# chg60/phamclust

Measured on AMD Instinct MI355X. Metric: genome-pairs/sec, higher is better.
Workload: dtype int32; 1 GPU; synth(5000,5000) -m peq: full N x N distance-matrix fill; `value` = fills with the genomes resident in HBM and the matrix left in HBM (upload and D2H excluded: see value_wall); n_genomes=5000, n_phams=5000, metric_selector=peq, genome_pairs=12497500, n_genes=531832, n_residues=111773410, parallelism=static pair shard over 1 GPU(s)

## Files before the change

### phamclust_amd/csrc/pc_align.hip

```cpp
#include <numeric>

#include "pc_host.h"

static int small_launch_min() {
    static const int v = [] { const char* e = getenv("PC_SMALL_LAUNCH_MIN"); const int x = e ? atoi(e) : 0; return x > 0 ? x : 192; }();
    return v;
}
static int run_align_classes(pc_ctx* c, const PcTask* task_list, const uint32_t* task_begin , const int32_t* cls_max_lb,
                             uint2* res, hipStream_t st, pc_stats* stats, int ppos) {
    const int nbase = c->ncls_all;
    struct Launch { uint32_t begin, end; int base, mode, max_lb; };
    std::vector<Launch> launches;
    for (int b = 0; b < nbase; ++b) {
        const uint32_t* tb = task_begin + (size_t)b * PC_WAVE_MODES;
        if (tb[PC_WAVE_MODES] == tb[0]) continue;
        const uint32_t n0 = tb[1] - tb[0], n1 = tb[2] - tb[1], n2 = tb[3] - tb[2];
        const int bv = pc_class_variant(b);
        const uint32_t least = (bv >= 0 && pc_nw_variant_w(bv) >= 32) ? 1u : (uint32_t)small_launch_min();
        const bool own2 = n2 >= least, own1 = n1 + (own2 ? 0u : n2) >= least;
        uint32_t at = tb[0];
        const int max_lb = cls_max_lb[b * PC_WAVE_MODES];
        auto put = [&](uint32_t n, int mode) { if (n) launches.push_back({at, at + n, b, mode, max_lb}); at += n; };
        if (own1) { put(n0, PC_MODE_CLASS); put(n1 + (own2 ? 0u : n2), n1 ? PC_MODE_TWO_WAVES : PC_MODE_ONE_WAVE); }
        else put(n0 + n1 + (own2 ? 0u : n2), n0 ? PC_MODE_CLASS : n1 ? PC_MODE_TWO_WAVES : PC_MODE_ONE_WAVE);
// ... 146 lines not shown

static int64_t plan_budget_bytes(pc_ctx* c) {
    if (c->plan_budget > 0) return c->plan_budget;
    size_t free_b = 0, total_b = 0;
    if (hipMemGetInfo(&free_b, &total_b) != hipSuccess) { (void)hipGetLastError(); return (int64_t)16 << 30; }
    const size_t held = c->b_key0.cap + c->b_key1.cap + c->b_val0.cap + c->b_val1.cap + c->b_flags.cap + c->b_excl.cap + c->b_alias.cap +
                        c->b_bucket_row.cap + c->b_res.cap + c->b_sort_tmp.cap;
    return (int64_t)((free_b + held) / 2);
}
static void release_plan_buffers(pc_ctx* c) {
    DevBuf* bufs[] = {&c->b_key0, &c->b_key1, &c->b_val0, &c->b_val1, &c->b_flags, &c->b_excl, &c->b_alias, &c->b_bucket_row, &c->b_res, &c->b_sort_tmp,
                      &c->b_tasks, &c->b_tasks_sorted};
    for (DevBuf* b : bufs) b->release();
}

static int stage_count(pc_ctx* c, int condensed, hipStream_t st, uint64_t tot[3]) {
    PcRange range("pc:count");
    int rc = PC_OK;
    const PcDev& d = c->dev;
    const int64_t Lp = c->shard_pairs;
    if (d.G > 0 && c->min_gene_len == 0) {
        pc_set_error("fill: an empty translation cannot be aligned (aai/peq); the reference fails on it too"); return PC_ERR_DATA;
    }
    if ((rc = c->b_na.ensure((Lp + 1) * 4)) || (rc = c->b_off.ensure((Lp + 1) * 4)) || (rc = c->b_totals.ensure(64))) return rc;
    PC_HIP(hipMemsetAsync(c->b_na.p, 0, (Lp + 1) * 4, st));
    PC_HIP(hipMemsetAsync(c->b_totals.p, 0, 64, st));
    PcWalkArgs a; memset(&a, 0, sizeof(a));
    a.na = c->b_na.as<uint32_t>(); a.totals = c->b_totals.as<unsigned long long>();
    a.as_distance = 0; a.condensed = condensed;
    if ((rc = pc_launch_walk(PCW_COUNT, d, c->shard, a, st))) return rc;
    uint64_t* h_tot = (uint64_t*)(c->h_plan.as<uint32_t>() + 1000);
    PC_HIP(hipMemcpyAsync(h_tot, c->b_totals.p, 24, hipMemcpyDeviceToHost, st));
    PC_HIP(hipStreamSynchronize(st));
    tot[0] = h_tot[0]; tot[1] = h_tot[1]; tot[2] = h_tot[2];
    return PC_OK;
}

static int count_per_target(pc_ctx* c, int condensed, hipStream_t st, std::vector<uint64_t>& per_owned) {
    int rc = PC_OK;
    const int N = c->dev.N;
    if ((rc = c->b_aln_t.ensure((size_t)N * 8))) return rc;
    PC_HIP(hipMemsetAsync(c->b_aln_t.p, 0, (size_t)N * 8, st));
    PcWalkArgs a; memset(&a, 0, sizeof(a));
    a.totals = c->b_totals.as<unsigned long long>() + 5;
    a.aln_t = c->b_aln_t.as<unsigned long long>(); a.condensed = condensed;
    if ((rc = pc_launch_walk(PCW_COUNT, c->dev, c->shard, a, st))) return rc;
    std::vector<uint64_t> all(N);
    PC_HIP(hipMemcpyAsync(all.data(), c->b_aln_t.p, (size_t)N * 8, hipMemcpyDeviceToHost, st));
    PC_HIP(hipStreamSynchronize(st));
// ... 26 lines not shown
    memset(&P.st, 0, sizeof(P.st));
    pc_stats& local = P.st;
    const int64_t base = (rows || groups) ? 0 : c->h_lbase[k0];
    const int64_t Lc = rows ? (int64_t)(k1 - k0) * d.N : groups ? groups->block_slot[k1] - groups->block_slot[k0] : c->h_lbase[k1] - base;
    local.n_pairs = Lc;
    local.n_alignments = (int64_t)A;
    if (A > (uint64_t)PC_PLAN_MAX_ALIGNMENTS) {
        pc_set_error("plan: %llu alignments behind ONE target genome exceed the 2^31-2 a plan can index", (unsigned long long)A); return PC_ERR_LIMIT;
    }
    const int U = d.U;
    const int ncls = c->nlc;
    const int64_t tmp_fixed = std::max<int64_t>(Lc + 1, U + 1);
    if ((rc = c->b_start_q.ensure((U + 1) * 4)) || (rc = c->b_end_q.ensure((U + 1) * 4)) || (rc = c->b_ntask_q.ensure((U + 1) * 4)) ||
        (rc = c->b_task_off_q.ensure((U + 1) * 4)) || (rc = c->b_scan_tmp.ensure(pc_scan_tmp_elems(tmp_fixed) * 4)) || (rc = c->b_plan.ensure(4096)))
        return rc;
    if (Lc > 0 && (rc = pc_scan_exclusive_u32(c->b_na.as<uint32_t>() + base, c->b_off.as<uint32_t>() + base, Lc, c->b_scan_tmp.as<uint32_t>(),
                                              (int64_t)(c->b_scan_tmp.cap / 4), st))) return rc;
    PcWalkArgs a; memset(&a, 0, sizeof(a));
    a.as_distance = 0; a.condensed = condensed;
    a.off = c->b_off.as<uint32_t>();
    uint32_t* const h_plan = c->h_plan.as<uint32_t>();
    uint64_t* h_tot = (uint64_t*)(h_plan + 1000);
    if (A > 0) {
        const int64_t An = (int64_t)A;
        const int key_bits = 2 * d.ubits;
        const size_t sort_bytes = pc_sort_temp_bytes(An, key_bits);
        if ((rc = c->b_key0.ensure(A * 8)) || (rc = c->b_key1.ensure(A * 8)) || (rc = c->b_val0.ensure(A * 4)) || (rc = c->b_val1.ensure(A * 4)) ||
            (rc = c->b_sort_tmp.ensure(std::max<size_t>(sort_bytes, 16))) || (rc = c->b_flags.ensure((A + 1) * 4)) || (rc = c->b_excl.ensure((A + 1) * 4)) ||
            (rc = c->b_alias.ensure(A * 4)) || (rc = c->b_bucket_row.ensure(A * 4)) || (rc = c->b_res.ensure(A * 8)) ||
            (rc = c->b_scan_tmp.ensure(pc_scan_tmp_elems(std::max<int64_t>(tmp_fixed, An + 1)) * 4)))
            return rc;
        const int64_t tmp_elems = (int64_t)(c->b_scan_tmp.cap / 4);
        a.key = c->b_key0.as<unsigned long long>(); a.val = c->b_val0.as<uint32_t>();
        if ((rc = walk_domain(c, PCW_ENUM, rows, groups, k0, k1, a, st))) return rc;
        if ((rc = pc_sort_pairs(c->b_sort_tmp.p, c->b_sort_tmp.cap, c->b_key0.as<unsigned long long>(), c->b_key1.as<unsigned long long>(),
                                c->b_val0.as<uint32_t>(), c->b_val1.as<uint32_t>(), An, key_bits, st))) return rc;
        if ((rc = pc_launch_mark_heads(c->b_key1.as<unsigned long long>(), c->b_flags.as<uint32_t>(), An, st))) return rc;
        if ((rc = pc_scan_exclusive_u32(c->b_flags.as<uint32_t>(), c->b_excl.as<uint32_t>(), An + 1, c->b_scan_tmp.as<uint32_t>(), tmp_elems, st))) return rc;
        PC_HIP(hipMemsetAsync(c->b_start_q.p, 0, (U + 1) * 4, st));
        PC_HIP(hipMemsetAsync(c->b_end_q.p, 0, (U + 1) * 4, st));
        PC_HIP(hipMemsetAsync(c->b_totals.as<unsigned long long>() + 3, 0, 16, st));
        if ((rc = pc_launch_unique(d, c->b_key1.as<unsigned long long>(), c->b_val1.as<uint32_t>(), c->b_flags.as<uint32_t>(), c->b_excl.as<uint32_t>(),
                                   c->b_alias.as<uint32_t>(), c->b_bucket_row.as<int32_t>(), c->b_start_q.as<uint32_t>(), c->b_end_q.as<uint32_t>(),
                                   c->b_totals.as<unsigned long long>(), An, st))) return rc;
        if ((rc = pc_launch_task_count(c->b_start_q.as<uint32_t>(), c->b_end_q.as<uint32_t>(), c->task_plan, c->b_ntask_q.as<uint32_t>(), U, st))) return rc;
        if ((rc = pc_scan_exclusive_u32(c->b_ntask_q.as<uint32_t>(), c->b_task_off_q.as<uint32_t>(), U + 1, c->b_scan_tmp.as<uint32_t>(), tmp_elems, st))) return rc;
        PC_HIP(hipMemcpyAsync(h_plan, c->b_task_off_q.as<uint32_t>() + U, 4, hipMemcpyDeviceToHost, st));
        PC_HIP(hipMemcpyAsync(h_tot, c->b_totals.p, 40, hipMemcpyDeviceToHost, st));
        PC_HIP(hipStreamSynchronize(st));
        const uint32_t ntasks = h_plan[0];
        local.n_tasks = ntasks; local.n_distinct_alignments = (int64_t)h_tot[3]; local.n_distinct_cells = (int64_t)h_tot[4];
        P.ntasks = ntasks; P.n_distinct = (int64_t)h_tot[3];
        int cbits = 1; while ((1 << cbits) < ncls) ++cbits;
        const size_t tb_bytes = pc_sort_temp_bytes((int64_t)std::max<uint32_t>(ntasks, 1), 32 + cbits);
        if ((rc = c->b_tasks.ensure(std::max<uint32_t>(ntasks, 1) * sizeof(PcTask))) || (rc = c->b_tasks_sorted.ensure(std::max<uint32_t>(ntasks, 1) * sizeof(PcTask))) ||
            (rc = c->b_key0.ensure((size_t)ntasks * 8)) || (rc = c->b_key1.ensure((size_t)ntasks * 8)) || (rc = c->b_val0.ensure((size_t)ntasks * 4)) ||
            (rc = c->b_val1.ensure((size_t)ntasks * 4)) || (rc = c->b_sort_tmp.ensure(std::max<size_t>(tb_bytes, 16))))
            return rc;
        if ((rc = pc_launch_task_fill(d, c->b_start_q.as<uint32_t>(), c->b_end_q.as<uint32_t>(), c->task_plan,
// ... 34 lines not shown
        PC_HIP(hipMemsetAsync(res, 0, (size_t)std::max<int64_t>(P.n_distinct, 1) * 8, st));
        task_list = c->b_tasks.as<PcTask>(); tb = sb;
    }
    for (int i = 0; i < ncls; ++i) c->aligned_tasks[i] = tb[i + 1] - tb[i];
    return run_align_classes(c, task_list, tb.data(), c->cls_max_lb.data(), res, st, stats, P.ppos);
}

static int stage_reduce(pc_ctx* c, int metric, int as_distance, const uint2* res, double* out, hipStream_t st, const PcRows* rows = nullptr,
                        const PcGroupsHost* groups = nullptr) {
    PcRange range("pc:reduce");
    pc_ctx::PlanState& P = c->plan;
    if (!P.valid) { pc_set_error("reduce: no plan (pc_plan_dev first)"); return PC_ERR_STATE; }
    PcWalkArgs a; memset(&a, 0, sizeof(a));
    a.off = c->b_off.as<uint32_t>(); a.alias = c->b_alias.as<uint32_t>(); a.res = res; a.out = out;
    a.as_distance = as_distance ? 1 : 0; a.condensed = P.condensed;
    return walk_domain(c, metric == PC_AAI ? PCW_AAI : PCW_PEQ, rows, groups, P.k0, P.k1, a, st);
}

static void add_plan_stats(pc_ctx* c, pc_stats& acc) {
    const pc_stats& ps = c->plan.st;
    acc.n_tasks += ps.n_tasks; acc.n_distinct_alignments += ps.n_distinct_alignments; acc.n_distinct_cells += ps.n_distinct_cells;
    for (size_t i = 0; i < c->aligned_tasks.size() && i < c->last_plan_tasks.size(); ++i) c->last_plan_tasks[i] += c->aligned_tasks[i];
}
static void set_last_plan_tasks(pc_ctx* c, const std::vector<uint32_t>& per_class) {
    c->last_plan_tasks.assign(per_class.begin(), per_class.end());
    c->last_plan_tasks.resize(c->nlc, 0);
    c->last_plan_tasks_valid = true;
}

static int chunk_step(pc_ctx* c, int metric, int ppos, int as_distance, int condensed, double* out, hipStream_t st, int k0, int k1, uint64_t A,
// ... 3 lines not shown
    if (rc == PC_OK) { if (events) PC_HIP(hipEventRecord(c->ev[2], st)); rc = stage_reduce(c, metric, as_distance, c->b_res.as<uint2>(), out, st, rows, groups); }
    if (rc != PC_OK) return rc;
    PC_HIP(hipEventRecord(c->ev[3], st));
    add_plan_stats(c, local);
    if (ms) {
        const hipEvent_t at[4] = {from, c->ev[1], c->ev[2], c->ev[3]};
        PC_HIP(hipEventSynchronize(c->ev[3]));
        for (int i = 0; i < 3; ++i) { float x = 0.f; PC_HIP(hipEventElapsedTime(&x, at[i], at[i + 1])); ms[i] += x; }
    }
    return PC_OK;
}
static int release_for_retry(pc_ctx* c, hipStream_t st, bool slots) {
    PC_HIP(hipStreamSynchronize(st));
    release_plan_buffers(c);
    c->b_scratch.release();
    if (slots) { c->b_na.release(); c->b_off.release(); }
    return PC_OK;
}

int fill_aligned(pc_ctx* c, int metric, int ppos, int as_distance, double* out, int condensed, hipStream_t st, pc_stats& local, bool timed) {
    int rc = PC_OK;
    if ((rc = fill_check_residues(c, "fill", metric))) return rc;
    uint64_t tot[3] = {0, 0, 0};
    c->last_plan_tasks_valid = false;
    c->last_plan_tasks.assign(c->nlc, 0);
    if ((rc = stage_count(c, condensed, st, tot))) return rc;
    local.n_alignments = (int64_t)tot[0]; local.n_cells = (int64_t)tot[1]; local.n_residue_bytes = (int64_t)tot[2];
    const int nown = c->shard.nown;
    const uint64_t A = tot[0];
    uint64_t max_aln = (uint64_t)PC_PLAN_MAX_ALIGNMENTS;
    if (c->plan_budget > 0 || A * PC_PLAN_BYTES_PER_ALIGNMENT > ((uint64_t)1 << 30))
// ... 36 lines not shown
}

static int fill_units_aligned(pc_ctx* c, const PcRows* rows, const PcGroupsHost* groups, int metric, int ppos, int as_distance, double* out,
                              hipStream_t st, pc_stats& local, bool timed) {
    int rc = PC_OK;
    const PcDev& d = c->dev;
    const int U = rows ? rows->nrows : groups->nblocks;
    auto slots = [&](int k0, int k1) { return rows ? (int64_t)(k1 - k0) * d.N : groups->block_slot[k1] - groups->block_slot[k0]; };
    if ((rc = fill_check_residues(c, "fill", metric))) return rc;
    if (d.G > 0 && c->min_gene_len == 0) {
        pc_set_error("fill: an empty translation cannot be aligned (aai/peq); the reference fails on it too"); return PC_ERR_DATA;
    }
    c->last_plan_tasks_valid = false;
    c->last_plan_tasks.assign(c->nlc, 0);
    c->plan.valid = false;
    std::vector<uint64_t> own(U);
    {
        PcRange range("pc:count");
        if ((rc = c->b_totals.ensure(64)) || (rc = c->b_aln_t.ensure((size_t)std::max(U, 1) * 8))) return rc;
        PC_HIP(hipMemsetAsync(c->b_totals.p, 0, 64, st));
        PC_HIP(hipMemsetAsync(c->b_aln_t.p, 0, (size_t)U * 8, st));
        PcWalkArgs a; memset(&a, 0, sizeof(a));
        a.totals = c->b_totals.as<unsigned long long>(); a.aln_t = c->b_aln_t.as<unsigned long long>();
        if ((rc = walk_domain(c, PCW_COUNT, rows, groups, 0, U, a, st))) return rc;
        uint64_t* h_tot = (uint64_t*)(c->h_plan.as<uint32_t>() + 1000);
        PC_HIP(hipMemcpyAsync(h_tot, c->b_totals.p, 24, hipMemcpyDeviceToHost, st));
        PC_HIP(hipMemcpyAsync(own.data(), c->b_aln_t.p, (size_t)U * 8, hipMemcpyDeviceToHost, st));
        PC_HIP(hipStreamSynchronize(st));
        local.n_alignments = (int64_t)h_tot[0]; local.n_cells = (int64_t)h_tot[1]; local.n_residue_bytes = (int64_t)h_tot[2];
    }
// ... 237 lines not shown
```

### phamclust_amd/csrc/pc_common.h

```cpp
#pragma once
#include <hip/hip_runtime.h>
#include <stdint.h>

#define PC_OPEN 11
#define PC_EXT 1
#define PC_NEG (-(1 << 29))
#define PC_PADCODE 255
#define PC_TASK_ROWS 208
#define PC_TASK_BUDGET 49152
#define PC_MAX_W 64

struct PcDev {
    int32_t N, Wb, Wstride, G;
    int32_t U, ubits;
    int32_t n_cu, pad_;
    int64_t E;
    const uint64_t* bitmap;
    const uint32_t* rankpre;
    const int32_t* ent_cnt;
    const int32_t* ent_len;
    const uint2* ent_pair_len;
    const uint2* ent_pair_cnt;
    const uint32_t* sp_end;
    const int32_t* sp_pham;
// ... 230 lines not shown
int pc_launch_affinity_rows_slab(const double* vals, int64_t Lp, const PcRowsSlab& dom, int r0, int n_rows, const int32_t* group, int G, void* state,
                                 int want_gain, hipEvent_t between, hipStream_t st);
int pc_launch_affinity_rows_finish(const void* state, const int32_t* rows, const int32_t* group, const int32_t* goff, const int32_t* qcount, int n_rows, int N,
                                   int G, int invert, void* out, int want_table, int want_gain, hipStream_t st);
struct PcLut { uint8_t v[256]; };
int pc_launch_encode(const uint8_t* raw, const int64_t* seq_off, const int64_t* gene_off, const int32_t* gene_len, const PcLut& lut,
                     uint8_t* codes, int G, hipStream_t st);
int pc_launch_task_keys(const PcDev& d, const PcTask* tasks, unsigned long long* key, uint32_t* val, int ntasks, hipStream_t st);
int pc_launch_task_gather(const PcTask* in, const uint32_t* idx, PcTask* out, int ntasks, hipStream_t st);
size_t pc_sort_temp_bytes(int64_t n, int bits);
int pc_sort_pairs(void* temp, size_t temp_bytes, const unsigned long long* key_in, unsigned long long* key_out, const uint32_t* val_in,
                  uint32_t* val_out, int64_t n, int bits, hipStream_t st);
int pc_launch_mark_heads(const unsigned long long* skey, uint32_t* flags, int64_t n, hipStream_t st);
int pc_launch_unique(const PcDev& d, const unsigned long long* skey, const uint32_t* sval, const uint32_t* flags, const uint32_t* excl,
                     uint32_t* alias, int32_t* bucket_row, uint32_t* start_q, uint32_t* end_q, unsigned long long* totals, int64_t n, hipStream_t st);
int pc_launch_task_count(const uint32_t* start_q, const uint32_t* end_q, const PcTaskPlan& tp, uint32_t* ntask_q, int U, hipStream_t st);
int pc_launch_task_fill(const PcDev& d, const uint32_t* start_q, const uint32_t* end_q, const PcTaskPlan& tp, const uint32_t* task_off_q,
                        PcTask* tasks, int U, hipStream_t st);
int pc_launch_class_bounds(const unsigned long long* sorted_key, int ntasks, int ncls, uint32_t* cls_begin , hipStream_t st);
int pc_launch_task_slice(const PcTask* sorted, int ntasks, const uint32_t* cls_begin, const uint32_t* slice_begin , int rank, int world,
                         PcTask* out, hipStream_t st);
int pc_launch_gather_u32(const uint32_t* src, const int32_t* idx, uint32_t* dst, int n, hipStream_t st);
int pc_launch_assemble(const double* gathered, int world, int64_t stride, int N, double* out, hipStream_t st);
int pc_launch_assemble_table(const double* gathered, int64_t stride, int N, const int32_t* t_rank, const int64_t* t_lbase, double* out, hipStream_t st);
int pc_launch_round6_probe(const double* in, double* out, int64_t n, hipStream_t st);
int pc_launch_unpack_res(const uint2* res, const int32_t* la_plus_lb, int32_t* n_ident, int32_t* n_diag, int64_t n, hipStream_t st);

int pc_nw_num_variants();
int pc_nw_variant_w(int v);
int pc_nw_choose_variant(int lb);
// ... 35 lines not shown
```

### phamclust_amd/csrc/pc_fill_slabs.hip

```cpp
#include <chrono>
#include <climits>

#include "pc_host.h"

#define PC_EDGE_MAX_PAIRS 0x7fffffffLL

namespace {
struct SlabShardScope {
    pc_ctx* c; PcShard shard; int64_t pairs; std::vector<int32_t> owned; std::vector<int64_t> lbase;
    explicit SlabShardScope(pc_ctx* ctx) : c(ctx), shard(ctx->shard), pairs(ctx->shard_pairs), owned(ctx->h_owned), lbase(ctx->h_lbase) {}
    ~SlabShardScope() { c->shard = shard; c->shard_pairs = pairs; c->h_owned.swap(owned); c->h_lbase.swap(lbase); c->plan.valid = false; }
    SlabShardScope(const SlabShardScope&) = delete; SlabShardScope& operator=(const SlabShardScope&) = delete;
};
}

static int64_t pairs_below(int64_t t) { return t * (t - 1) / 2; }

int pc_slab_check(const pc_ctx* c, PcSlabRun& run, const char* what) {
    int rc = PC_OK;
    const char* who = run.who;
    if ((rc = fill_check(c, who, what, &run.metric, nullptr))) return rc;
    if (run.kind == PC_SLAB_NEAREST) {
        if (run.k < 1) { pc_set_error("%s: k %d", who, run.k); return PC_ERR_ARG; }
        if (run.k > PC_NEAREST_MAX_K) { pc_set_error("%s: k %d is above PC_NEAREST_MAX_K = %d", who, run.k, PC_NEAREST_MAX_K); return PC_ERR_LIMIT; }
        run.kk = std::max(std::min(run.k, c->dev.N - 1), 0);
    }
// ... 62 lines not shown
template <class Hook> static int slab_walk(pc_ctx* c, const std::vector<int32_t>& cut, int metric, int as_distance, pc_stats* sum, Hook hook) {
    int rc = PC_OK;
    hipStream_t st = c->stream;
    double* const slab = c->b_edge_slab.as<double>();
    SlabShardScope restore(c);
    std::vector<int32_t> owned; std::vector<int64_t> lbase;
    for (size_t i = 0; i + 1 < cut.size(); ++i) {
        const int t0 = cut[i], t1 = cut[i + 1];
        const int64_t Lp = pairs_below(t1) - pairs_below(t0);
        if (Lp == 0) continue;
        owned.resize((size_t)(t1 - t0)); lbase.resize((size_t)(t1 - t0) + 1);
        for (int t = t0; t < t1; ++t) { owned[t - t0] = t; lbase[t - t0] = pairs_below(t) - pairs_below(t0); }
        lbase[t1 - t0] = Lp;
        if ((rc = wait_last_work(c, st, false))) return rc;
        if ((rc = upload_vec(c->b_edge_owned, owned)) || (rc = upload_vec(c->b_edge_lbase, lbase))) return rc;
        c->plan.valid = false;
        c->shard.nown = t1 - t0; c->shard.ident = 0;
        c->shard.owned = c->b_edge_owned.as<int32_t>(); c->shard.lbase = c->b_edge_lbase.as<int64_t>();
        c->h_owned = owned; c->h_lbase = lbase; c->shard_pairs = Lp;
        pc_stats one; memset(&one, 0, sizeof(one));
        if ((rc = fill_impl(c, metric, as_distance, slab, 0, st, sum ? &one : nullptr))) return rc;
        if (sum) pc_stats_add(*sum, one);
        int64_t hooked_pairs = 0;
        if (const double* const hooked = pc_hooked_slab_values(&hooked_pairs)) {
            if (hooked_pairs != pairs_below(c->dev.N)) {
                pc_set_error("slab walk: pc_hook_slab_values holds %lld values, the triangle of %d genomes has %lld", (long long)hooked_pairs, c->dev.N,
                             (long long)pairs_below(c->dev.N));
                return PC_ERR_ARG;
            }
            PC_HIP(hipMemcpyAsync(slab, hooked + pairs_below(t0), (size_t)Lp * 8, hipMemcpyHostToDevice, st));
        }
// ... 1098 lines not shown
```

### phamclust_amd/csrc/pc_host.h

```cpp
#pragma once
#include <algorithm>
#include <cstdint>
#include <cstdlib>
#include <cstring>
#include <thread>
#include <vector>

#include "pc_common.h"
#include "pc_nw_geometry.h"
#include "../../include/phamclust_hip.h"

struct PcRange {
    bool on;
    explicit PcRange(const char* name);
    ~PcRange();
    PcRange(const PcRange&) = delete; PcRange& operator=(const PcRange&) = delete;
};

constexpr int PC_ERR_NOMEM_INTERNAL = -100;
struct PlanningScope { PlanningScope(); ~PlanningScope(); };
__attribute__((visibility("hidden"))) const double* pc_hooked_slab_values(int64_t* n_pairs);
__attribute__((visibility("hidden"))) const double* pc_hooked_rows_values(int32_t* n_rows, int32_t* n);
struct DevBuf {
    void* p = nullptr; size_t cap = 0;
// ... 100 lines not shown
    DevBuf b_af_group, b_af_member, b_af_goff, b_af_range, b_af_tab, b_af_out, b_af_qcount;
    PinnedBuf h_af;
    int af_ranges = 0;
    float last_af_ms[3] = {0.f, 0.f, 0.f};
    DevBuf b_hist_group, b_hist_state, b_hist_out;
    PinnedBuf h_hist;
    float last_hist_ms[2] = {0.f, 0.f};
    PinnedBuf h_plan;
    struct PlanState {
        bool valid = false; int ppos = 0; int condensed = 1; int64_t A = 0, n_distinct = 0; uint32_t ntasks = 0;
        int k0 = 0, k1 = 0;
        bool whole = false;
        std::vector<uint32_t> tb;
        pc_stats st;
    } plan;
    std::vector<uint32_t> aligned_tasks;
    std::vector<int64_t> last_plan_tasks;
    bool last_plan_tasks_valid = false;
    PinnedBuf h_out;
    float last_align_ms = 0.f;
    hipEvent_t ev[5] = {nullptr, nullptr, nullptr, nullptr, nullptr};
    static constexpr int kAux = 15;
    hipStream_t aux[kAux] = {};
    hipEvent_t aux_ev[kAux + 1] = {};
    int n_streams = 8;
    static constexpr int kLong = 4;
    hipStream_t lng[kLong] = {};
    hipEvent_t lng_ev[kLong] = {};
    int tie_rule = 0;
    int64_t lut_key = -1; const double* lut_ptr = nullptr;
    hipEvent_t ev_last = nullptr;
    bool busy = false;
    hipStream_t last_stream = nullptr;
    int last_set_kernel = -1;
    pc_set_inputs last_set_inputs{};
    pc_set_shape last_set_shape{};
    int64_t plan_budget = 0;
};

struct PcDeviceGuard {
    int prev = -1, dev = -1; bool ok = true;
    explicit PcDeviceGuard(int device) : dev(device) {
        if (hipGetDevice(&prev) != hipSuccess) prev = -1;
        if (prev != dev) {
            hipError_t e = hipSetDevice(dev);
            if (e != hipSuccess) { pc_set_error("hipSetDevice(%d): %s", dev, hipGetErrorString(e)); ok = false; }
        }
    }
    ~PcDeviceGuard() { if (prev >= 0 && prev != dev) (void)hipSetDevice(prev); }
    PcDeviceGuard(const PcDeviceGuard&) = delete;
    PcDeviceGuard& operator=(const PcDeviceGuard&) = delete;
};
#define PC_ON_DEVICE(c) PcDeviceGuard pc_guard_((c)->device); if (!pc_guard_.ok) return PC_ERR_HIP
// ... 209 lines not shown
```

### phamclust_amd/csrc/pc_plan.hip

```cpp
#include <cstring>

#include <rocprim/device/device_radix_sort.hpp>

#include "../../include/phamclust_hip.h"
#include "pc_common.h"
#include "pc_nw_geometry.h"

size_t pc_sort_temp_bytes(int64_t n, int bits) {
    size_t bytes = 0;
    if (n <= 0) return 0;
    hipError_t e = rocprim::radix_sort_pairs(nullptr, bytes, (const unsigned long long*)nullptr, (unsigned long long*)nullptr,
                                             (const uint32_t*)nullptr, (uint32_t*)nullptr, (size_t)n, 0u, (unsigned)bits, (hipStream_t)0);
    return e == hipSuccess ? bytes : 0;
}

int pc_sort_pairs(void* temp, size_t temp_bytes, const unsigned long long* key_in, unsigned long long* key_out, const uint32_t* val_in,
                  uint32_t* val_out, int64_t n, int bits, hipStream_t st) {
    if (n <= 0) return PC_OK;
    hipError_t e = rocprim::radix_sort_pairs(temp, temp_bytes, key_in, key_out, val_in, val_out, (size_t)n, 0u, (unsigned)bits, st);
    if (e != hipSuccess) { pc_set_error("radix_sort_pairs: %s", hipGetErrorString(e)); return PC_ERR_HIP; }
    return PC_OK;
}

__global__ __launch_bounds__(256) void k_mark_heads(const unsigned long long* __restrict__ skey, uint32_t* __restrict__ flags, int64_t n) {
// ... 36 lines not shown
    }
    for (int o = 32; o > 0; o >>= 1) { cells += __shfl_down(cells, o); heads += __shfl_down(heads, o); }
    if ((threadIdx.x & 63) == 0 && heads) { atomicAdd(&red[0], heads); atomicAdd(&red[1], cells); }
    __syncthreads();
    if (threadIdx.x < 2 && red[threadIdx.x]) atomicAdd(&totals[3 + threadIdx.x], red[threadIdx.x]);
}
int pc_launch_unique(const PcDev& d, const unsigned long long* skey, const uint32_t* sval, const uint32_t* flags, const uint32_t* excl,
                     uint32_t* alias, int32_t* bucket_row, uint32_t* start_q, uint32_t* end_q, unsigned long long* totals, int64_t n, hipStream_t st) {
    if (n <= 0) return PC_OK;
    hipLaunchKernelGGL(k_unique, dim3((unsigned)((n + 255) / 256)), dim3(256), 0, st, d, skey, sval, flags, excl, alias, bucket_row, start_q, end_q, totals, n);
    hipError_t e = hipGetLastError();
    if (e != hipSuccess) { pc_set_error("k_unique launch: %s", hipGetErrorString(e)); return PC_ERR_HIP; }
    return PC_OK;
}

__device__ __forceinline__ uint32_t pc_split(const PcTaskPlan& tp, int q, uint32_t n, uint32_t& rem_class) {
    const uint32_t nseg = tp.q_nseg[q], r = nseg > 1 ? n % nseg : 0u;
    rem_class = r ? tp.rem_class[(size_t)q * 16 + r] : 255u;
    return rem_class != 255u ? n - r : n;
}
__global__ void k_task_count(const uint32_t* __restrict__ start_q, const uint32_t* __restrict__ end_q, PcTaskPlan tp,
                             uint32_t* __restrict__ ntask_q, int U) {
    const int q = blockIdx.x * blockDim.x + threadIdx.x;
    if (q > U) return;
    uint32_t nt = 0;
    if (q < U) {
        const uint32_t n = end_q[q] - start_q[q], per = (uint32_t)tp.task_rows[q];
        uint32_t rc; const uint32_t nmain = pc_split(tp, q, n, rc);
        nt = (nmain + per - 1) / per + (rc != 255u ? 1u : 0u);
    }
// ... 112 lines not shown
```

### phamclust_amd/csrc/pc_upload.hip

```cpp
#include <atomic>
#include <chrono>
#include <cstdio>
#include <mutex>
#include <numeric>

#include "pc_host.h"

static void build_code_lut(uint8_t lut[256]) {
    static const char alpha[] = "ARNDCQEGHILKMFPSTWYVBZX*";
    int assigned[256];
    for (int i = 0; i < 256; ++i) assigned[i] = -1;
    for (int k = 0; k < 24; ++k) assigned[(unsigned char)alpha[k]] = k;
    int next = 24;
    for (int v = 0; v < 256; ++v) {
        if (v >= 'a' && v <= 'z') continue;
        if (assigned[v] < 0) assigned[v] = next++;
    }
    for (int v = 'a'; v <= 'z'; ++v) assigned[v] = assigned[v - 32];
    for (int i = 0; i < 256; ++i) lut[i] = (uint8_t)assigned[i];
}

static int apply_shard(pc_ctx* c, int rank, int world) {
    c->plan.valid = false;
    const int N = c->dev.N;
    std::vector<int32_t> owned; std::vector<int64_t> lbase;
    c->h_t_rank.assign(std::max(N, 1), 0); c->h_t_lbase.assign(std::max(N, 1), 0);
    int64_t best = 0;
    for (int r = 0; r < world; ++r) {
        int64_t tot = 0;
        for (int j = 0;; ++j) {
            const int pos = (j & 1) ? world - 1 - r : r;
            const int64_t t = (int64_t)j * world + pos;
            if (t >= N) { if ((int64_t)j * world >= N) break; else continue; }
            if (r == rank) { owned.push_back((int32_t)t); lbase.push_back(tot); }
            c->h_t_rank[t] = r; c->h_t_lbase[t] = tot;
            tot += t;
        }
        if (r == rank) { lbase.push_back(tot); c->shard_pairs = tot; }
// ... 21 lines not shown
    }
    const int64_t G64 = g->gene_off[N];
    if (G64 < 0 || G64 > 0x7fffffffLL || g->gene_off[0] != 0 || (G64 > 0 && (!g->gene_pham || !g->residues))) {
        pc_set_error("pc_upload: bad gene table"); return PC_ERR_ARG;
    }
    const int G = (int)G64;
    static const bool timing = getenv("PC_UPLOAD_TIMING") != nullptr;
    auto tick = std::chrono::steady_clock::now();
    auto lap = [&](const char* what) {
        if (!timing) return;
        auto now = std::chrono::steady_clock::now();
        fprintf(stderr, "pc_upload %-22s %7.1f ms\n", what, std::chrono::duration<double, std::milli>(now - tick).count());
        tick = now;
    };
    if ((rc = wait_last_work(c, nullptr, false))) return rc;
    c->uploaded = false; c->residues_ready = false; c->target_cost.clear(); c->plan.valid = false;
    PC_HIP(hipStreamSynchronize(c->stream));
    if (c->b_scratch.cap > ((size_t)512 << 20)) c->b_scratch.release();

    const int Wstride = W | 1;
    size_t off = 0;
    auto place = [&](size_t bytes) { const size_t at = off; off = (off + bytes + 255) & ~(size_t)255; return at; };
    const size_t o_bitmap = place((size_t)N * Wstride * 8), o_rankpre = place((size_t)N * W * 4), o_gene_len = place((size_t)std::max(G, 1) * 4),
                 o_ent_off = place(((size_t)N + 1) * 4), o_nph = place((size_t)N * 4), o_ngen = place((size_t)N * 4), o_tlen = place((size_t)N * 8);
    const size_t o_ent = off;
    const size_t cap_bytes = o_ent + 6 * (((size_t)std::max(G, 1) * 4 + 255) & ~(size_t)255) + (((size_t)N + 1) * 4 + 255) + (size_t)std::max(P, 1) * 4 + 1024;
    if ((rc = c->h_stage.ensure(cap_bytes))) return rc;
    uint8_t* hs = c->h_stage.as<uint8_t>();
    uint64_t* bitmap = (uint64_t*)(hs + o_bitmap); uint32_t* rankpre = (uint32_t*)(hs + o_rankpre); int32_t* gene_len_h = (int32_t*)(hs + o_gene_len);
    uint32_t* ent_off = (uint32_t*)(hs + o_ent_off); int32_t* nph_h = (int32_t*)(hs + o_nph); int32_t* ngen_h = (int32_t*)(hs + o_ngen);
    int64_t* tlen_h = (int64_t*)(hs + o_tlen);
// ... 165 lines not shown
    const int N = g->n_genomes;
    const int G = c->dev.G;
    if (N != c->dev.N || g->gene_off[N] != (int64_t)G || g->seq_off[G] - g->seq_off[0] != c->n_residue_bytes_in) {
        pc_set_error("pc_upload_residues: not the genomes pc_upload_sets was given (N %d/%d, genes %lld/%d)", N, c->dev.N, (long long)g->gene_off[N], G);
        return PC_ERR_ARG;
    }
    static const bool timing = getenv("PC_UPLOAD_TIMING") != nullptr;
    auto tick = std::chrono::steady_clock::now();
    auto lap = [&](const char* what) {
        if (!timing) return;
        auto now = std::chrono::steady_clock::now();
        fprintf(stderr, "pc_upload %-22s %7.1f ms\n", what, std::chrono::duration<double, std::milli>(now - tick).count());
        tick = now;
    };
    if ((rc = wait_last_work(c, nullptr, false))) return rc;
    c->residues_ready = false; c->plan.valid = false;
    PC_HIP(hipStreamSynchronize(c->stream));
    const std::vector<int32_t>& gene_len = c->h_gene_len;
    const int maxlen = c->max_gene_len;
    std::vector<int64_t> gene_off(G);
    int64_t code_bytes = 0;
    for (int k = 0; k < G; ++k) { gene_off[k] = code_bytes; code_bytes += ((int64_t)gene_len[k] + 15) & ~15LL; }
    std::vector<uint64_t> ghash(std::max(G, 1));
    std::vector<uint8_t> godd(std::max(G, 1), 0);
    uint8_t lut[256]; build_code_lut(lut);
    uint8_t is_odd[256];
    for (int v = 0; v < 256; ++v) is_odd[v] = (uint8_t)(lut[v] >= 24);
    const uint8_t* raw = g->residues;
    const int64_t raw_bytes = g->seq_off[G] - g->seq_off[0];
    static const int64_t stage_max = getenv("PC_RAW_STAGE_MAX") ? atoll(getenv("PC_RAW_STAGE_MAX")) : ((int64_t)512 << 20);
    const bool staged = raw_bytes > 0 && raw_bytes <= stage_max;
// ... 284 lines not shown
    std::vector<int64_t> t_lbase(std::max(N, 1), 0), fill(world, 0);
    std::vector<int32_t> owned; std::vector<int64_t> lbase;
    for (int t = 0; t < N; ++t) {
        const int r = t_rank[t];
        t_lbase[t] = fill[r];
        if (r == rank) { owned.push_back(t); lbase.push_back(fill[r]); }
        fill[r] += t;
    }
    lbase.push_back(fill[rank]);
    c->shard_pairs = fill[rank];
    c->shard_stride = *std::max_element(fill.begin(), fill.end());
    c->rank = rank; c->world = world; c->balanced = true;
    if ((rc = upload_vec(c->b_owned, owned)) || (rc = upload_vec(c->b_lbase, lbase)) || (rc = upload_vec(c->b_t_rank, t_rank)) ||
        (rc = upload_vec(c->b_t_lbase, t_lbase))) return rc;
    c->h_t_rank = t_rank; c->h_t_lbase = t_lbase;
    c->h_owned = owned; c->h_lbase = lbase; c->plan.valid = false;
    c->shard.nown = (int32_t)owned.size();
    c->shard.ident = world == 1 ? 1 : 0;
    c->shard.owned = c->b_owned.as<int32_t>();
    c->shard.lbase = c->b_lbase.as<int64_t>();
    return PC_OK;
}
extern "C" int pc_shard_table(const pc_ctx* c, int32_t* t_rank, int64_t* t_lbase) {
    if (!c || !c->uploaded) { pc_set_error("pc_shard_table: upload first"); return PC_ERR_STATE; }
    if (!t_rank || !t_lbase) { pc_set_error("pc_shard_table: NULL argument"); return PC_ERR_ARG; }
    memcpy(t_rank, c->h_t_rank.data(), sizeof(int32_t) * (size_t)c->dev.N);
    memcpy(t_lbase, c->h_t_lbase.data(), sizeof(int64_t) * (size_t)c->dev.N);
    return PC_OK;
}
extern "C" int pc_target_costs(const pc_ctx* c, uint64_t* cost) {
    if (!c || !c->uploaded) { pc_set_error("pc_target_costs: upload first"); return PC_ERR_STATE; }
// ... 8 lines not shown
```

### phamclust_amd/csrc/pc_walk.hip

```cpp
#include "pc_pairs.h"

#define WCH 32

struct PcPairAcc {
    uint32_t k;
    int64_t cons;
    double num;
    int64_t den;
    int any;
    __device__ __forceinline__ void reset() { k = 0; cons = 0; num = 0.0; den = 0; any = 0; }
};

template <int MODE>
__device__ __forceinline__ void pc_visit(const PcDev& d, const PcWalkArgs& a, PcPairAcc& p, uint32_t es, uint32_t et,
                                         unsigned long long& cells, unsigned long long& rbytes) {
    p.any = 1;
    if (MODE == PCW_POCP) { p.cons += d.ent_cnt[es] + d.ent_cnt[et]; return; }
    if (MODE == PCW_AF) { p.cons += d.ent_len[es] + d.ent_len[et]; return; }
    const int cs = d.ent_cnt[es], ct = d.ent_cnt[et];
    const bool swap = cs > ct;
    const uint32_t ea = swap ? et : es, eb = swap ? es : et;
    const int ca = swap ? ct : cs, cb = swap ? cs : ct;
    const int a0 = d.ent_gene[ea], b0 = d.ent_gene[eb];
    if (MODE == PCW_COUNT) {
// ... 4 lines not shown
        rbytes += la * cb + lb * ca;
    } else if (MODE == PCW_ENUM) {
        for (int ia = 0; ia < ca; ++ia) {
            const unsigned long long qa = d.gene_q[a0 + ia];
            for (int ib = 0; ib < cb; ++ib) {
                const uint32_t k = p.k++;
                a.key[k] = ((unsigned long long)d.gene_q[b0 + ib] << d.ubits) | qa;
                a.val[k] = k;
            }
        }
    } else {
        if (MODE == PCW_PEQ) p.cons += d.ent_len[es] + d.ent_len[et];
        for (int ia = 0; ia < ca; ++ia) {
            double best = -1.0; uint32_t best_len = 0;
            for (int ib = 0; ib < cb; ++ib) {
                const uint2 r = a.res[a.alias[p.k++]];
                const double x = (double)r.x / (double)r.y;
                if (x >= best) { best = x; best_len = r.y; }
            }
            p.num = p.num + best * (double)best_len;
            p.den += best_len;
        }
    }
}

template <int MODE>
__device__ __forceinline__ void pc_walk_word(const PcDev& d, const PcWalkArgs& a, PcPairAcc& acc, uint64_t sw, uint64_t tw, uint32_t bs, uint32_t bt,
                                             unsigned long long& cells, unsigned long long& rbytes) {
    uint64_t x = sw & tw;
    while (x) {
        const int b = __ffsll((long long)x) - 1;
// ... 355 lines not shown
```

Baseline: 25.21 million genome-pairs/s.

## Cache pair counts across fills, fuse unique pass, pre-gather alignment results

The per-pair count walk and its offset scan are now cached on the context and reused by later fills. The cache is invalidated whenever the shard, upload or residues change, which removes a full walk over all genome pairs from each repeated fill. Head marking, the flag scan and unique assignment are replaced by a block-level head count, a small scan and one fused kernel, cutting passes over the sorted keys. Before the reduce walk, alignment results are gathered into slot order so the PEQ/AAI walk reads them contiguously instead of through the alias indirection, at the cost of one extra gather kernel.

```diff
diff --git a/phamclust_amd/csrc/pc_align.hip b/phamclust_amd/csrc/pc_align.hip
--- a/phamclust_amd/csrc/pc_align.hip
+++ b/phamclust_amd/csrc/pc_align.hip
@@ -184,6 +184,8 @@
     for (DevBuf* b : bufs) b->release();
 }
 
+static bool plan_switch(const char* name) { const char* e = getenv(name); return !(e && !strcmp(e, "0")); }
+
 static int stage_count(pc_ctx* c, int condensed, hipStream_t st, uint64_t tot[3]) {
     PcRange range("pc:count");
     int rc = PC_OK;
@@ -192,6 +194,12 @@
     if (d.G > 0 && c->min_gene_len == 0) {
         pc_set_error("fill: an empty translation cannot be aligned (aai/peq); the reference fails on it too"); return PC_ERR_DATA;
     }
+    pc_ctx::CountState& C = c->count;
+    if (C.valid && C.condensed == condensed && plan_switch("PC_COUNT_ONCE") && c->b_na.cap >= (size_t)(Lp + 1) * 4 && c->b_off.cap >= (size_t)(Lp + 1) * 4) {
+        tot[0] = C.tot[0]; tot[1] = C.tot[1]; tot[2] = C.tot[2];
+        return PC_OK;
+    }
+    C.valid = C.off_valid = false;
     if ((rc = c->b_na.ensure((Lp + 1) * 4)) || (rc = c->b_off.ensure((Lp + 1) * 4)) || (rc = c->b_totals.ensure(64))) return rc;
     PC_HIP(hipMemsetAsync(c->b_na.p, 0, (Lp + 1) * 4, st));
     PC_HIP(hipMemsetAsync(c->b_totals.p, 0, 64, st));
@@ -203,6 +211,7 @@
     PC_HIP(hipMemcpyAsync(h_tot, c->b_totals.p, 24, hipMemcpyDeviceToHost, st));
     PC_HIP(hipStreamSynchronize(st));
     tot[0] = h_tot[0]; tot[1] = h_tot[1]; tot[2] = h_tot[2];
+    C.valid = true; C.condensed = condensed; C.tot[0] = tot[0]; C.tot[1] = tot[1]; C.tot[2] = tot[2];
     return PC_OK;
 }
 
@@ -259,8 +268,13 @@
     if ((rc = c->b_start_q.ensure((U + 1) * 4)) || (rc = c->b_end_q.ensure((U + 1) * 4)) || (rc = c->b_ntask_q.ensure((U + 1) * 4)) ||
         (rc = c->b_task_off_q.ensure((U + 1) * 4)) || (rc = c->b_scan_tmp.ensure(pc_scan_tmp_elems(tmp_fixed) * 4)) || (rc = c->b_plan.ensure(4096)))
         return rc;
-    if (Lc > 0 && (rc = pc_scan_exclusive_u32(c->b_na.as<uint32_t>() + base, c->b_off.as<uint32_t>() + base, Lc, c->b_scan_tmp.as<uint32_t>(),
-                                              (int64_t)(c->b_scan_tmp.cap / 4), st))) return rc;
+    const bool whole_shard = !rows && !groups && k0 == 0 && k1 == c->shard.nown && c->count.valid && c->count.condensed == condensed;
+    if (!(whole_shard && c->count.off_valid && plan_switch("PC_COUNT_ONCE"))) {
+        c->count.off_valid = false;
+        if (Lc > 0 && (rc = pc_scan_exclusive_u32(c->b_na.as<uint32_t>() + base, c->b_off.as<uint32_t>() + base, Lc, c->b_scan_tmp.as<uint32_t>(),
+                                                  (int64_t)(c->b_scan_tmp.cap / 4), st))) return rc;
+        c->count.off_valid = whole_shard;
+    }
     PcWalkArgs a; memset(&a, 0, sizeof(a));
     a.as_distance = 0; a.condensed = condensed;
     a.off = c->b_off.as<uint32_t>();
@@ -270,8 +284,10 @@
         const int64_t An = (int64_t)A;
         const int key_bits = 2 * d.ubits;
         const size_t sort_bytes = pc_sort_temp_bytes(An, key_bits);
+        const bool fused = plan_switch("PC_PLAN_FUSED");
+        const size_t flag_words = fused ? (size_t)pc_unique_blocks(An) + 1 : (size_t)A + 1;
         if ((rc = c->b_key0.ensure(A * 8)) || (rc = c->b_key1.ensure(A * 8)) || (rc = c->b_val0.ensure(A * 4)) || (rc = c->b_val1.ensure(A * 4)) ||
-            (rc = c->b_sort_tmp.ensure(std::max<size_t>(sort_bytes, 16))) || (rc = c->b_flags.ensure((A + 1) * 4)) || (rc = c->b_excl.ensure((A + 1) * 4)) ||
+            (rc = c->b_sort_tmp.ensure(std::max<size_t>(sort_bytes, 16))) || (rc = c->b_flags.ensure(flag_words * 4)) || (rc = c->b_excl.ensure(flag_words * 4)) ||
             (rc = c->b_alias.ensure(A * 4)) || (rc = c->b_bucket_row.ensure(A * 4)) || (rc = c->b_res.ensure(A * 8)) ||
             (rc = c->b_scan_tmp.ensure(pc_scan_tmp_elems(std::max<int64_t>(tmp_fixed, An + 1)) * 4)))
             return rc;
@@ -280,14 +296,20 @@
         if ((rc = walk_domain(c, PCW_ENUM, rows, groups, k0, k1, a, st))) return rc;
         if ((rc = pc_sort_pairs(c->b_sort_tmp.p, c->b_sort_tmp.cap, c->b_key0.as<unsigned long long>(), c->b_key1.as<unsigned long long>(),
                                 c->b_val0.as<uint32_t>(), c->b_val1.as<uint32_t>(), An, key_bits, st))) return rc;
-        if ((rc = pc_launch_mark_heads(c->b_key1.as<unsigned long long>(), c->b_flags.as<uint32_t>(), An, st))) return rc;
-        if ((rc = pc_scan_exclusive_u32(c->b_flags.as<uint32_t>(), c->b_excl.as<uint32_t>(), An + 1, c->b_scan_tmp.as<uint32_t>(), tmp_elems, st))) return rc;
         PC_HIP(hipMemsetAsync(c->b_start_q.p, 0, (U + 1) * 4, st));
         PC_HIP(hipMemsetAsync(c->b_end_q.p, 0, (U + 1) * 4, st));
         PC_HIP(hipMemsetAsync(c->b_totals.as<unsigned long long>() + 3, 0, 16, st));
-        if ((rc = pc_launch_unique(d, c->b_key1.as<unsigned long long>(), c->b_val1.as<uint32_t>(), c->b_flags.as<uint32_t>(), c->b_excl.as<uint32_t>(),
-                                   c->b_alias.as<uint32_t>(), c->b_bucket_row.as<int32_t>(), c->b_start_q.as<uint32_t>(), c->b_end_q.as<uint32_t>(),
-                                   c->b_totals.as<unsigned long long>(), An, st))) return rc;
+        if (fused) {
+            if ((rc = pc_launch_unique_fused(d, c->b_key1.as<unsigned long long>(), c->b_val1.as<uint32_t>(), c->b_flags.as<uint32_t>(), c->b_excl.as<uint32_t>(),
+                                             c->b_scan_tmp.as<uint32_t>(), tmp_elems, c->b_alias.as<uint32_t>(), c->b_bucket_row.as<int32_t>(),
+                                             c->b_start_q.as<uint32_t>(), c->b_end_q.as<uint32_t>(), c->b_totals.as<unsigned long long>(), An, st))) return rc;
+        } else {
+            if ((rc = pc_launch_mark_heads(c->b_key1.as<unsigned long long>(), c->b_flags.as<uint32_t>(), An, st))) return rc;
+            if ((rc = pc_scan_exclusive_u32(c->b_flags.as<uint32_t>(), c->b_excl.as<uint32_t>(), An + 1, c->b_scan_tmp.as<uint32_t>(), tmp_elems, st))) return rc;
+            if ((rc = pc_launch_unique(d, c->b_key1.as<unsigned long long>(), c->b_val1.as<uint32_t>(), c->b_flags.as<uint32_t>(), c->b_excl.as<uint32_t>(),
+                                       c->b_alias.as<uint32_t>(), c->b_bucket_row.as<int32_t>(), c->b_start_q.as<uint32_t>(), c->b_end_q.as<uint32_t>(),
+                                       c->b_totals.as<unsigned long long>(), An, st))) return rc;
+        }
         if ((rc = pc_launch_task_count(c->b_start_q.as<uint32_t>(), c->b_end_q.as<uint32_t>(), c->task_plan, c->b_ntask_q.as<uint32_t>(), U, st))) return rc;
         if ((rc = pc_scan_exclusive_u32(c->b_ntask_q.as<uint32_t>(), c->b_task_off_q.as<uint32_t>(), U + 1, c->b_scan_tmp.as<uint32_t>(), tmp_elems, st))) return rc;
         PC_HIP(hipMemcpyAsync(h_plan, c->b_task_off_q.as<uint32_t>() + U, 4, hipMemcpyDeviceToHost, st));
@@ -352,6 +374,11 @@
     PcWalkArgs a; memset(&a, 0, sizeof(a));
     a.off = c->b_off.as<uint32_t>(); a.alias = c->b_alias.as<uint32_t>(); a.res = res; a.out = out;
     a.as_distance = as_distance ? 1 : 0; a.condensed = P.condensed;
+    if (P.A > 0 && plan_switch("PC_REDUCE_GATHER") && c->b_key0.cap >= (size_t)P.A * 8) {
+        int rc = pc_launch_gather_results(a.alias, res, c->b_key0.as<uint2>(), P.A, st);
+        if (rc != PC_OK) return rc;
+        a.alias = nullptr; a.res = c->b_key0.as<uint2>();
+    }
     return walk_domain(c, metric == PC_AAI ? PCW_AAI : PCW_PEQ, rows, groups, P.k0, P.k1, a, st);
 }
 
@@ -385,7 +412,7 @@
     PC_HIP(hipStreamSynchronize(st));
     release_plan_buffers(c);
     c->b_scratch.release();
-    if (slots) { c->b_na.release(); c->b_off.release(); }
+    if (slots) { c->b_na.release(); c->b_off.release(); c->count.valid = c->count.off_valid = false; }
     return PC_OK;
 }
 
@@ -452,6 +479,7 @@
     c->last_plan_tasks_valid = false;
     c->last_plan_tasks.assign(c->nlc, 0);
     c->plan.valid = false;
+    c->count.valid = c->count.off_valid = false;
     std::vector<uint64_t> own(U);
     {
         PcRange range("pc:count");
diff --git a/phamclust_amd/csrc/pc_common.h b/phamclust_amd/csrc/pc_common.h
--- a/phamclust_amd/csrc/pc_common.h
+++ b/phamclust_amd/csrc/pc_common.h
@@ -268,6 +268,11 @@
 int pc_launch_mark_heads(const unsigned long long* skey, uint32_t* flags, int64_t n, hipStream_t st);
 int pc_launch_unique(const PcDev& d, const unsigned long long* skey, const uint32_t* sval, const uint32_t* flags, const uint32_t* excl,
                      uint32_t* alias, int32_t* bucket_row, uint32_t* start_q, uint32_t* end_q, unsigned long long* totals, int64_t n, hipStream_t st);
+int64_t pc_unique_blocks(int64_t n);
+int pc_launch_unique_fused(const PcDev& d, const unsigned long long* skey, const uint32_t* sval, uint32_t* block_heads, uint32_t* block_off,
+                           uint32_t* tmp, int64_t tmp_elems, uint32_t* alias, int32_t* bucket_row, uint32_t* start_q, uint32_t* end_q,
+                           unsigned long long* totals, int64_t n, hipStream_t st);
+int pc_launch_gather_results(const uint32_t* alias, const uint2* res, uint2* slot_res , int64_t n, hipStream_t st);
 int pc_launch_task_count(const uint32_t* start_q, const uint32_t* end_q, const PcTaskPlan& tp, uint32_t* ntask_q, int U, hipStream_t st);
 int pc_launch_task_fill(const PcDev& d, const uint32_t* start_q, const uint32_t* end_q, const PcTaskPlan& tp, const uint32_t* task_off_q,
                         PcTask* tasks, int U, hipStream_t st);
diff --git a/phamclust_amd/csrc/pc_fill_slabs.hip b/phamclust_amd/csrc/pc_fill_slabs.hip
--- a/phamclust_amd/csrc/pc_fill_slabs.hip
+++ b/phamclust_amd/csrc/pc_fill_slabs.hip
@@ -9,7 +9,7 @@
 struct SlabShardScope {
     pc_ctx* c; PcShard shard; int64_t pairs; std::vector<int32_t> owned; std::vector<int64_t> lbase;
     explicit SlabShardScope(pc_ctx* ctx) : c(ctx), shard(ctx->shard), pairs(ctx->shard_pairs), owned(ctx->h_owned), lbase(ctx->h_lbase) {}
-    ~SlabShardScope() { c->shard = shard; c->shard_pairs = pairs; c->h_owned.swap(owned); c->h_lbase.swap(lbase); c->plan.valid = false; }
+    ~SlabShardScope() { c->shard = shard; c->shard_pairs = pairs; c->h_owned.swap(owned); c->h_lbase.swap(lbase); pc_shard_changed(c); }
     SlabShardScope(const SlabShardScope&) = delete; SlabShardScope& operator=(const SlabShardScope&) = delete;
 };
 }
@@ -102,7 +102,7 @@
         lbase[t1 - t0] = Lp;
         if ((rc = wait_last_work(c, st, false))) return rc;
         if ((rc = upload_vec(c->b_edge_owned, owned)) || (rc = upload_vec(c->b_edge_lbase, lbase))) return rc;
-        c->plan.valid = false;
+        pc_shard_changed(c);
         c->shard.nown = t1 - t0; c->shard.ident = 0;
         c->shard.owned = c->b_edge_owned.as<int32_t>(); c->shard.lbase = c->b_edge_lbase.as<int64_t>();
         c->h_owned = owned; c->h_lbase = lbase; c->shard_pairs = Lp;
diff --git a/phamclust_amd/csrc/pc_host.h b/phamclust_amd/csrc/pc_host.h
--- a/phamclust_amd/csrc/pc_host.h
+++ b/phamclust_amd/csrc/pc_host.h
@@ -138,6 +138,9 @@
         std::vector<uint32_t> tb;
         pc_stats st;
     } plan;
+    struct CountState {
+        bool valid = false, off_valid = false; int condensed = 1; uint64_t tot[3] = {0, 0, 0};
+    } count;
     std::vector<uint32_t> aligned_tasks;
     std::vector<int64_t> last_plan_tasks;
     bool last_plan_tasks_valid = false;
@@ -161,6 +164,8 @@
     pc_set_shape last_set_shape{};
     int64_t plan_budget = 0;
 };
+
+static inline void pc_shard_changed(pc_ctx* c) { c->plan.valid = false; c->count.valid = c->count.off_valid = false; }
 
 struct PcDeviceGuard {
     int prev = -1, dev = -1; bool ok = true;
diff --git a/phamclust_amd/csrc/pc_plan.hip b/phamclust_amd/csrc/pc_plan.hip
--- a/phamclust_amd/csrc/pc_plan.hip
+++ b/phamclust_amd/csrc/pc_plan.hip
@@ -74,6 +74,114 @@
     return PC_OK;
 }
 
+#define PC_UNIQ_PER_BLOCK 2048
+__device__ __forceinline__ uint32_t pc_load_heads(const unsigned long long* __restrict__ skey, int64_t base, int64_t n, unsigned long long k[8],
+                                                  unsigned long long& prev) {
+    if (base >= n) return 0u;
+    if (base + 8 <= n) {
+        const ulonglong2* p = (const ulonglong2*)(skey + base);
+#pragma unroll
+        for (int i = 0; i < 4; ++i) { const ulonglong2 v = p[i]; k[2 * i] = v.x; k[2 * i + 1] = v.y; }
+    } else {
+#pragma unroll
+        for (int i = 0; i < 8; ++i) k[i] = base + i < n ? skey[base + i] : 0ull;
+    }
+    prev = base > 0 ? skey[base - 1] : ~k[0];
+    uint32_t bits = 0;
+#pragma unroll
+    for (int i = 0; i < 8; ++i) if (base + i < n && k[i] != (i ? k[i - 1] : prev)) bits |= 1u << i;
+    return bits;
+}
+__global__ __launch_bounds__(256) void k_head_count(const unsigned long long* __restrict__ skey, uint32_t* __restrict__ block_heads, int64_t n) {
+    __shared__ uint32_t wsum[4];
+    unsigned long long k[8], prev;
+    uint32_t cnt = (uint32_t)__popc(pc_load_heads(skey, (int64_t)blockIdx.x * PC_UNIQ_PER_BLOCK + (int64_t)threadIdx.x * 8, n, k, prev));
+    for (int o = 32; o > 0; o >>= 1) cnt += __shfl_down(cnt, o);
+    if ((threadIdx.x & 63) == 0) wsum[threadIdx.x >> 6] = cnt;
+    __syncthreads();
+    if (threadIdx.x == 0) block_heads[blockIdx.x] = wsum[0] + wsum[1] + wsum[2] + wsum[3];
+}
+__global__ __launch_bounds__(256) void k_unique_fused(PcDev d, const unsigned long long* __restrict__ skey, const uint32_t* __restrict__ sval,
+                                                      const uint32_t* __restrict__ block_off, uint32_t* __restrict__ alias,
+                                                      int32_t* __restrict__ bucket_row, uint32_t* __restrict__ start_q, uint32_t* __restrict__ end_q,
+                                                      unsigned long long* __restrict__ totals, int64_t n) {
+    __shared__ uint32_t wsum[4];
+    __shared__ unsigned long long red[2];
+    if (threadIdx.x < 2) red[threadIdx.x] = 0;
+    const int64_t base = (int64_t)blockIdx.x * PC_UNIQ_PER_BLOCK + (int64_t)threadIdx.x * 8;
+    unsigned long long k[8], prev = 0;
+    const uint32_t bits = pc_load_heads(skey, base, n, k, prev);
+    uint32_t v[8];
+    if (base + 8 <= n) {
+        const uint4 a = ((const uint4*)(sval + base))[0], b = ((const uint4*)(sval + base))[1];
+        v[0] = a.x; v[1] = a.y; v[2] = a.z; v[3] = a.w; v[4] = b.x; v[5] = b.y; v[6] = b.z; v[7] = b.w;
+    } else {
+#pragma unroll
+        for (int i = 0; i < 8; ++i) v[i] = base + i < n ? sval[base + i] : 0u;
+    }
+    const uint32_t tot = (uint32_t)__popc(bits);
+    uint32_t incl = tot;
+    const int lane = threadIdx.x & 63, wv = threadIdx.x >> 6;
+#pragma unroll
+    for (int o = 1; o < 64; o <<= 1) { const uint32_t y = __shfl_up(incl, o); if (lane >= o) incl += y; }
+    if (lane == 63) wsum[wv] = incl;
+    __syncthreads();
+    uint32_t run = block_off[blockIdx.x] + incl - tot;
+    for (int i = 0; i < wv; ++i) run += wsum[i];
+    unsigned long long cells = 0, heads = 0;
+    const unsigned long long qmask = (1ull << d.ubits) - 1;
+#pragma unroll
+    for (int i = 0; i < 8; ++i) {
+        if (base + i >= n) break;
+        const uint32_t f = (bits >> i) & 1u, u = run + f - 1u;
+        run += f;
+        alias[v[i]] = u;
+        const uint32_t qb = (uint32_t)(k[i] >> d.ubits);
+        if (f) {
+            const int ga = d.q_gene[(uint32_t)(k[i] & qmask)];
+            bucket_row[u] = ga;
+            cells += (unsigned long long)d.gene_len[ga] * (unsigned long long)d.gene_len[d.q_gene[qb]];
+            heads += 1;
+            if (base + i == 0) start_q[qb] = 0;
+            else {
+                const uint32_t qp = (uint32_t)((i ? k[i - 1] : prev) >> d.ubits);
+                if (qp != qb) { start_q[qb] = u; end_q[qp] = u; }
+            }
+        }
+        if (base + i == n - 1) end_q[qb] = u + 1;
+    }
+    for (int o = 32; o > 0; o >>= 1) { cells += __shfl_down(cells, o); heads += __shfl_down(heads, o); }
+    if (lane == 0 && heads) { atomicAdd(&red[0], heads); atomicAdd(&red[1], cells); }
+    __syncthreads();
+    if (threadIdx.x < 2 && red[threadIdx.x]) atomicAdd(&totals[3 + threadIdx.x], red[threadIdx.x]);
+}
+int64_t pc_unique_blocks(int64_t n) { return n > 0 ? (n + PC_UNIQ_PER_BLOCK - 1) / PC_UNIQ_PER_BLOCK : 0; }
+int pc_launch_unique_fused(const PcDev& d, const unsigned long long* skey, const uint32_t* sval, uint32_t* block_heads, uint32_t* block_off,
+                           uint32_t* tmp, int64_t tmp_elems, uint32_t* alias, int32_t* bucket_row, uint32_t* start_q, uint32_t* end_q,
+                           unsigned long long* totals, int64_t n, hipStream_t st) {
+    if (n <= 0) return PC_OK;
+    const int64_t nb = pc_unique_blocks(n);
+    hipLaunchKernelGGL(k_head_count, dim3((unsigned)nb), dim3(256), 0, st, skey, block_heads, n);
+    int rc = pc_scan_exclusive_u32(block_heads, block_off, nb, tmp, tmp_elems, st);
+    if (rc != PC_OK) return rc;
+    hipLaunchKernelGGL(k_unique_fused, dim3((unsigned)nb), dim3(256), 0, st, d, skey, sval, block_off, alias, bucket_row, start_q, end_q, totals, n);
+    hipError_t e = hipGetLastError();
+    if (e != hipSuccess) { pc_set_error("k_unique_fused launch: %s", hipGetErrorString(e)); return PC_ERR_HIP; }
+    return PC_OK;
+}
+
+__global__ __launch_bounds__(256) void k_gather_results(const uint32_t* __restrict__ alias, const uint2* __restrict__ res, uint2* __restrict__ slot_res, int64_t n) {
+    const int64_t k = (int64_t)blockIdx.x * blockDim.x + threadIdx.x;
+    if (k < n) slot_res[k] = res[alias[k]];
+}
+int pc_launch_gather_results(const uint32_t* alias, const uint2* res, uint2* slot_res, int64_t n, hipStream_t st) {
+    if (n <= 0) return PC_OK;
+    hipLaunchKernelGGL(k_gather_results, dim3((unsigned)((n + 255) / 256)), dim3(256), 0, st, alias, res, slot_res, n);
+    hipError_t e = hipGetLastError();
+    if (e != hipSuccess) { pc_set_error("k_gather_results launch: %s", hipGetErrorString(e)); return PC_ERR_HIP; }
+    return PC_OK;
+}
+
 __device__ __forceinline__ uint32_t pc_split(const PcTaskPlan& tp, int q, uint32_t n, uint32_t& rem_class) {
     const uint32_t nseg = tp.q_nseg[q], r = nseg > 1 ? n % nseg : 0u;
     rem_class = r ? tp.rem_class[(size_t)q * 16 + r] : 255u;
diff --git a/phamclust_amd/csrc/pc_upload.hip b/phamclust_amd/csrc/pc_upload.hip
--- a/phamclust_amd/csrc/pc_upload.hip
+++ b/phamclust_amd/csrc/pc_upload.hip
@@ -21,7 +21,7 @@
 }
 
 static int apply_shard(pc_ctx* c, int rank, int world) {
-    c->plan.valid = false;
+    pc_shard_changed(c);
     const int N = c->dev.N;
     std::vector<int32_t> owned; std::vector<int64_t> lbase;
     c->h_t_rank.assign(std::max(N, 1), 0); c->h_t_lbase.assign(std::max(N, 1), 0);
@@ -73,7 +73,7 @@
         tick = now;
     };
     if ((rc = wait_last_work(c, nullptr, false))) return rc;
-    c->uploaded = false; c->residues_ready = false; c->target_cost.clear(); c->plan.valid = false;
+    c->uploaded = false; c->residues_ready = false; c->target_cost.clear(); pc_shard_changed(c);
     PC_HIP(hipStreamSynchronize(c->stream));
     if (c->b_scratch.cap > ((size_t)512 << 20)) c->b_scratch.release();
 
@@ -269,7 +269,7 @@
         tick = now;
     };
     if ((rc = wait_last_work(c, nullptr, false))) return rc;
-    c->residues_ready = false; c->plan.valid = false;
+    c->residues_ready = false; pc_shard_changed(c);
     PC_HIP(hipStreamSynchronize(c->stream));
     const std::vector<int32_t>& gene_len = c->h_gene_len;
     const int maxlen = c->max_gene_len;
@@ -584,7 +584,7 @@
     if ((rc = upload_vec(c->b_owned, owned)) || (rc = upload_vec(c->b_lbase, lbase)) || (rc = upload_vec(c->b_t_rank, t_rank)) ||
         (rc = upload_vec(c->b_t_lbase, t_lbase))) return rc;
     c->h_t_rank = t_rank; c->h_t_lbase = t_lbase;
-    c->h_owned = owned; c->h_lbase = lbase; c->plan.valid = false;
+    c->h_owned = owned; c->h_lbase = lbase; pc_shard_changed(c);
     c->shard.nown = (int32_t)owned.size();
     c->shard.ident = world == 1 ? 1 : 0;
     c->shard.owned = c->b_owned.as<int32_t>();
diff --git a/phamclust_amd/csrc/pc_walk.hip b/phamclust_amd/csrc/pc_walk.hip
--- a/phamclust_amd/csrc/pc_walk.hip
+++ b/phamclust_amd/csrc/pc_walk.hip
@@ -42,7 +42,8 @@
         for (int ia = 0; ia < ca; ++ia) {
             double best = -1.0; uint32_t best_len = 0;
             for (int ib = 0; ib < cb; ++ib) {
-                const uint2 r = a.res[a.alias[p.k++]];
+                const uint32_t k = p.k++;
+                const uint2 r = a.alias ? a.res[a.alias[k]] : a.res[k];
                 const double x = (double)r.x / (double)r.y;
                 if (x >= best) { best = x; best_len = r.y; }
             }
```

Result: no change. 25.29 million genome-pairs/s, median of 6 (+0.3%).
